# Keep-Passion/ImageStitch

Hardware: AMD Instinct MI355X
Metric: image-pairs/sec (2048x2048 grayscale, SURF+BF) (higher is better)
Workload: dtype f32

## Files before the change

### imagestitch_amd/csrc/match_kernels.hip

```cpp
#include "common.h"
#include <algorithm>
#include <stdlib.h>
#include <math.h>

typedef float float2v __attribute__((ext_vector_type(2)));
typedef const float __attribute__((address_space(4))) cfloat;
typedef float f16v __attribute__((ext_vector_type(16)));

#define SLOAD16(dst, ptr) asm volatile("s_load_dwordx16 %0, %1, 0x0" : "=s"(dst) : "s"(ptr))
#define SLOAD16_BEFORE(dst, ptr, live) asm volatile("s_load_dwordx16 %0, %2, 0x0" : "=s"(dst), "+s"(live) : "s"(ptr))
#define SWAIT(dst) asm volatile("s_waitcnt lgkmcnt(0)" : "+s"(dst))
#define SWAIT2(d0, d1) asm volatile("s_waitcnt lgkmcnt(0)" : "+s"(d0), "+s"(d1))
#define BF_CHUNK(buf, base)                                                                    \
    _Pragma("unroll") for (int d = 0; d < 16; d += 4) {                                        \
        float2v e0 = qv[base + d + 0] - buf[d + 0];                                            \
        float2v e1 = qv[base + d + 1] - buf[d + 1];                                            \
        float2v e2 = qv[base + d + 2] - buf[d + 2];                                            \
        float2v e3 = qv[base + d + 3] - buf[d + 3];                                            \
        acc += e0 * e0 + e1 * e1 + e2 * e2 + e3 * e3;                                          \
    }

__device__ __forceinline__ void knn_update(float dsq, int j, float &b1, float &b2, int &i1, float &b1sq, float &b2sq)
{
    if (dsq < b2sq) {
// ... 134 lines not shown
    float b1[4], b2[4], b1s[4], b2s[4];
#pragma unroll
    for (int u = 0; u < 4; u++) {
        const int q = qw + 16 * u + c;
        const i4v *qp = (const i4v *)(J.q8 + (size_t)q * 128);
        qb[u][0] = qp[g]; qb[u][1] = qp[4 + g];
        qn[u] = J.qn2[q];
        thr[u] = 0x7fffffff; i1[u] = -1;
        b1[u] = b2[u] = b1s[u] = b2s[u] = INFINITY;
    }
    for (int jt = t0; jt < t1; jt += 16) {
        const i4v *tp = (const i4v *)(J.t8 + (size_t)(jt + c) * 128);
        const i4v a0 = tp[g], a1 = tp[4 + g];
        const i4v tn = *(const i4v *)(J.tn2 + jt + 4 * g);
        const int j0 = jt + 4 * g;
#pragma unroll
        for (int u = 0; u < 4; u++) {
            i4v acc = {0, 0, 0, 0};
            acc = __builtin_amdgcn_mfma_i32_16x16x64_i8(a0, qb[u][0], acc, 0, 0, 0);
            acc = __builtin_amdgcn_mfma_i32_16x16x64_i8(a1, qb[u][1], acc, 0, 0, 0);
            const int s0 = tn[0] - 2 * acc[0], s1 = tn[1] - 2 * acc[1], s2 = tn[2] - 2 * acc[2], s3 = tn[3] - 2 * acc[3];
            if (min(min(s0, s1), min(s2, s3)) < thr[u]) {
                if (s0 < thr[u] && j0 < nt) knn_update((float)(s0 + qn[u]), j0, b1[u], b2[u], i1[u], b1s[u], b2s[u]);
                if (s1 < thr[u] && j0 + 1 < nt) knn_update((float)(s1 + qn[u]), j0 + 1, b1[u], b2[u], i1[u], b1s[u], b2s[u]);
                if (s2 < thr[u] && j0 + 2 < nt) knn_update((float)(s2 + qn[u]), j0 + 2, b1[u], b2[u], i1[u], b1s[u], b2s[u]);
                if (s3 < thr[u] && j0 + 3 < nt) knn_update((float)(s3 + qn[u]), j0 + 3, b1[u], b2[u], i1[u], b1s[u], b2s[u]);
                thr[u] = b2s[u] == INFINITY ? 0x7fffffff : (int)b2s[u] - qn[u];
            }
        }
    }
    const size_t o = (size_t)sp * J.capq;
#pragma unroll
    for (int u = 0; u < 4; u++) {
        float B1 = b1[u], B2 = b2[u]; int I1 = i1[u];
#pragma unroll
        for (int d = 16; d <= 32; d <<= 1) {
            const float ob1 = __shfl_xor(B1, d, 64), ob2 = __shfl_xor(B2, d, 64);
            const int oi1 = __shfl_xor(I1, d, 64);
            knn_merge(B1, B2, I1, ob1, ob2, oi1);
        }
        const int q = qw + 16 * u + c;
        if (g == 0 && q < nq) { J.p_d1[o + q] = B1; J.p_d2[o + q] = B2; J.p_i1[o + q] = I1; }
    }
}

#define BFM_CAPL 32
#define BFM_MARGIN 1e-3f
#define BFM_FAR 1e30f

struct BfmState { float m1, m2, thr; int cnt; };

__device__ __forceinline__ void bfm_warm(const f16v &acc, BfmState &S)
{
#pragma unroll
    for (int i = 0; i < 16; i++) {
        const float v = acc[i];
        S.m2 = fminf(S.m2, fmaxf(S.m1, v));
        S.m1 = fminf(S.m1, v);
    }
}
__device__ __forceinline__ void bfm_scan(const f16v &acc, BfmState &S, int row0, uint2 *list, size_t pitch, bool update)
{
#pragma unroll
    for (int i = 0; i < 16; i++) {
        const float v = acc[i];
        if (v <= S.thr && v < 1e29f) {
            if (S.cnt < BFM_CAPL) list[S.cnt * pitch] = make_uint2(__float_as_uint(v), (unsigned)(row0 + (i & 3) + 8 * (i >> 2)));
            S.cnt++;
            if (update) {
                S.m2 = fminf(S.m2, fmaxf(S.m1, v));
                S.m1 = fminf(S.m1, v);
                S.thr = S.m2 + BFM_MARGIN;
            }
        }
    }
}

__global__ __launch_bounds__(256, 2) void k_bf_mfma_d64(const MatchDev *jobs)
{
    const MatchDev &J = jobs[blockIdx.z];
    const int nq = __builtin_amdgcn_readfirstlane(*J.nq_ptr), nt = __builtin_amdgcn_readfirstlane(*J.nt_ptr);
    const int lane = threadIdx.x & 63, wave = threadIdx.x >> 6;
    const int q0 = (blockIdx.x * 4 + wave) * 64;
    if (q0 >= nq) return;
    const int nsplit = gridDim.y, sp = blockIdx.y;
    const int ntiles = (nt + 31) >> 5;
    const int tchunk = (ntiles + nsplit - 1) / nsplit;
    const int tile0 = sp * tchunk, tile1 = min(ntiles, tile0 + tchunk);
    const int col = lane & 31, half = lane >> 5;
    float bq0[32], bq1[32];
    {
        const float4 *p0 = reinterpret_cast<const float4 *>(J.q + (size_t)min(q0 + col, nq - 1) * 64 + 32 * half);
        const float4 *p1 = reinterpret_cast<const float4 *>(J.q + (size_t)min(q0 + 32 + col, nq - 1) * 64 + 32 * half);
#pragma unroll
        for (int s4 = 0; s4 < 8; s4++) {
            const float4 u = p0[s4], v = p1[s4];
            bq0[4 * s4 + 0] = -2.f * u.x; bq0[4 * s4 + 1] = -2.f * u.y; bq0[4 * s4 + 2] = -2.f * u.z; bq0[4 * s4 + 3] = -2.f * u.w;
            bq1[4 * s4 + 0] = -2.f * v.x; bq1[4 * s4 + 1] = -2.f * v.y; bq1[4 * s4 + 2] = -2.f * v.z; bq1[4 * s4 + 3] = -2.f * v.w;
        }
    }
    const float baug = half == 0 ? 1.f : 0.f;
    const bool va = q0 + col < nq, vb = q0 + 32 + col < nq;
    BfmState Sa = {INFINITY, INFINITY, INFINITY, 0}, Sb = {INFINITY, INFINITY, INFINITY, 0};
    const size_t pitch = (size_t)J.capq;
    const int lst = sp * 2 + half;
    uint2 *lista = J.c_ent + (size_t)lst * BFM_CAPL * pitch + (q0 + col), *listb = lista + 32;
    const float *T = J.t;
    for (int pass = 0; pass < 2; pass++) {
        const int tend = pass == 0 ? min(tile0 + 1, tile1) : tile1;
        float4 an[8];
        if (tile0 < tend) {
            const float4 *pn = reinterpret_cast<const float4 *>(T + (size_t)min(tile0 * 32 + col, nt - 1) * 64 + 32 * half);
#pragma unroll
            for (int s4 = 0; s4 < 8; s4++) an[s4] = pn[s4];
        }
        for (int tl = tile0; tl < tend; tl++) {
            float a[32];
#pragma unroll
            for (int s4 = 0; s4 < 8; s4++) { a[4 * s4] = an[s4].x; a[4 * s4 + 1] = an[s4].y; a[4 * s4 + 2] = an[s4].z; a[4 * s4 + 3] = an[s4].w; }
            if (tl + 1 < tend) {
                const float4 *pn = reinterpret_cast<const float4 *>(T + (size_t)min((tl + 1) * 32 + col, nt - 1) * 64 + 32 * half);
#pragma unroll
                for (int s4 = 0; s4 < 8; s4++) an[s4] = pn[s4];
            }
            float part = 0.f;
#pragma unroll
            for (int s = 0; s < 32; s++) part += a[s] * a[s];
            const float tnorm = part + __shfl_xor(part, 32, 64);
            const float aaug = half == 0 ? (tl * 32 + col < nt ? tnorm : BFM_FAR) : 0.f;
            f16v acc0 = {0, 0, 0, 0, 0, 0, 0, 0, 0, 0, 0, 0, 0, 0, 0, 0}, acc1 = acc0;
#pragma unroll
            for (int s = 0; s < 32; s++) {
                acc0 = __builtin_amdgcn_mfma_f32_32x32x2f32(a[s], bq0[s], acc0, 0, 0, 0);
                acc1 = __builtin_amdgcn_mfma_f32_32x32x2f32(a[s], bq1[s], acc1, 0, 0, 0);
            }
            acc0 = __builtin_amdgcn_mfma_f32_32x32x2f32(aaug, baug, acc0, 0, 0, 0);
            acc1 = __builtin_amdgcn_mfma_f32_32x32x2f32(aaug, baug, acc1, 0, 0, 0);
            if (pass == 0) {
                bfm_warm(acc0, Sa); bfm_warm(acc1, Sb);
            } else {
                const int row0 = tl * 32 + 4 * half;
                bfm_scan(acc0, Sa, row0, lista, pitch, tl != tile0); bfm_scan(acc1, Sb, row0, listb, pitch, tl != tile0);
            }
        }
        if (pass == 0) {
            Sa.thr = va ? Sa.m2 + BFM_MARGIN : -INFINITY;
            Sb.thr = vb ? Sb.m2 + BFM_MARGIN : -INFINITY;
        }
    }
    if (va) J.c_cnt[(size_t)lst * pitch + q0 + col] = Sa.cnt;
    if (vb) J.c_cnt[(size_t)lst * pitch + q0 + 32 + col] = Sb.cnt;
}

#define BF16_ROW 80
#define BF16_FRAGS 5
#define BFM_F16_ERR 2.0e-3f
typedef _Float16 h8v __attribute__((ext_vector_type(8)));

__global__ __launch_bounds__(256) void k_bf_split16(const MatchDev *jobs, float scale_q)
{
    const MatchDev &J = jobs[blockIdx.z];
    const bool is_t = blockIdx.y == 1;
    const int n = is_t ? *J.nt_ptr : *J.nq_ptr;
    const int row = blockIdx.x * 128 + (threadIdx.x >> 1), half = threadIdx.x & 1;
    if (row >= n) return;
    const float *src = (is_t ? J.t : J.q) + (size_t)row * 64 + 32 * half;
    const float sc = is_t ? 1.f : scale_q;
    float part = 0.f;
    h8v el[4];
#pragma unroll
    for (int d = 0; d < 32; d++) {
        const float x = src[d];
        part += x * x;
        el[d >> 3][d & 7] = (_Float16)(x * sc);
    }
    const float tot = part + __shfl_xor(part, 1, 64);
    h8v ns = {0, 0, 0, 0, 0, 0, 0, 0};
    if (half == 0) {
        _Float16 a = (_Float16)1.f, b = (_Float16)1.f;
        if (is_t) { a = (_Float16)tot; b = (_Float16)(tot - (float)a); }
        ns[0] = a; ns[1] = b;
    }
    if (is_t) {
        h8v *dst = reinterpret_cast<h8v *>(J.t16) + (size_t)(row >> 5) * (BF16_FRAGS * 64) + (row & 31) + 32 * half;
#pragma unroll
        for (int s4 = 0; s4 < 4; s4++) dst[s4 * 64] = el[s4];
        dst[4 * 64] = ns;
    } else {
        h8v *dst = reinterpret_cast<h8v *>(J.q16 + (size_t)row * BF16_ROW + 32 * half);
#pragma unroll
        for (int s4 = 0; s4 < 4; s4++) dst[s4] = el[s4];
        if (half == 0) *reinterpret_cast<h8v *>(J.q16 + (size_t)row * BF16_ROW + 64) = ns;
    }
}

#ifndef BFM_GLDS
#define BFM_GLDS 1
#endif
#define BFM_WINDOW (2.f * BFM_F16_ERR + BFM_MARGIN)
#define GASM __attribute__((address_space(1)))
typedef GASM const h8v *g_cs8v;
typedef float f2v __attribute__((ext_vector_type(2)));

#ifdef VFSMS_DESC_TIMING
__device__ unsigned long long g_bf_cycles[2][8];
extern "C" int vfsms_debug_bf_cycles(unsigned long long *out) { return hipMemcpyFromSymbol(out, HIP_SYMBOL(g_bf_cycles), sizeof(unsigned long long) * 16) == hipSuccess ? 0 : -3; }
#define BT_DECL unsigned long long _bt[5] = {0, 0, 0, 0, 0}, _bt0 = clock64(), _btl = _bt0
#define BT_MARK(ph) do { const unsigned long long _n = clock64(); _bt[ph] += _n - _btl; _btl = _n; } while (0)
#define BT_FLUSH(pass) do { if ((threadIdx.x & 63) == 0) { for (int _q = 0; _q < 5; _q++) atomicAdd(&g_bf_cycles[pass][_q], _bt[_q]); \
        atomicAdd(&g_bf_cycles[pass][5], clock64() - _bt0); atomicAdd(&g_bf_cycles[pass][6], 1ull); } } while (0)
#else
#define BT_DECL do {} while (0)
#define BT_MARK(ph) do {} while (0)
#define BT_FLUSH(pass) do {} while (0)
#endif
template <int PASS>
__global__ __launch_bounds__(256, 3) void k_bf_mfma16_d64(const MatchDev *jobs, int qblocks, int nsplit, int njobs)
{
    unsigned unit, qb;
    xcd_roi_map(blockIdx.x, (unsigned)qblocks, (unsigned)(nsplit * njobs), unit, qb);
    const int sp = (int)(unit % (unsigned)nsplit);
    const MatchDev &J = jobs[unit / (unsigned)nsplit];
    const int nq = __builtin_amdgcn_readfirstlane(*J.nq_ptr), nt = __builtin_amdgcn_readfirstlane(*J.nt_ptr);
    const int lane = threadIdx.x & 63, wave = threadIdx.x >> 6;
    if ((int)qb * 256 >= nq) return;
    BT_DECL;
    const int q0 = ((int)qb * 4 + wave) * 64;
    const bool live = q0 < nq;
    const int ntiles = (nt + 31) >> 5;
    const int tchunk = (ntiles + nsplit - 1) / nsplit;
    const int tile0 = sp * tchunk, tile1 = min(ntiles, tile0 + tchunk);
    const int col = lane & 31, half = lane >> 5;
    const h8v zero = {0, 0, 0, 0, 0, 0, 0, 0};
    h8v bh0[4], bh1[4], bn0, bn1;
    {
        g_cs8v p0 = (g_cs8v)(J.q16 + (size_t)min(q0 + col, nq - 1) * BF16_ROW + 32 * half);
        g_cs8v p1 = (g_cs8v)(J.q16 + (size_t)min(q0 + 32 + col, nq - 1) * BF16_ROW + 32 * half);
#pragma unroll
        for (int s4 = 0; s4 < 4; s4++) { bh0[s4] = p0[s4]; bh1[s4] = p1[s4]; }
        bn0 = half == 0 ? *(g_cs8v)(J.q16 + (size_t)min(q0 + col, nq - 1) * BF16_ROW + 64) : zero;
        bn1 = half == 0 ? *(g_cs8v)(J.q16 + (size_t)min(q0 + 32 + col, nq - 1) * BF16_ROW + 64) : zero;
    }
    constexpr int NFR = BF16_FRAGS;
    constexpr int BFM_UNIT = 2;
    __shared__ h8v stage[2][BFM_UNIT][NFR * 64];
    g_cs8v T = (g_cs8v)J.t16;
    const int tid = threadIdx.x; (void)tid;
#if BFM_GLDS
    constexpr int NSET = 1;
    const int wv_u = __builtin_amdgcn_readfirstlane(wave);
    auto glds16 = [&](g_cs8v src, const h8v *dst) {
        __builtin_amdgcn_global_load_lds((const __attribute__((address_space(1))) void *)src, (__attribute__((address_space(3))) void *)dst, 16, 0, 0);
    };
    auto fetch = [&](int unit, int b) {
#pragma unroll
        for (int u = 0; u < BFM_UNIT; u++) {
            const int tl = min(tile0 + unit * BFM_UNIT + u, tile1 - 1);
            g_cs8v pn = T + (size_t)tl * (BF16_FRAGS * 64);
            glds16(pn + 64 * wv_u + lane, &stage[b][u][64 * wv_u]);
            if (wv_u == 0) glds16(pn + 256 + lane, &stage[b][u][256]);
        }
    };
    const int nunits = (tile1 - tile0 + BFM_UNIT - 1) / BFM_UNIT;
    if (nunits > 0) fetch(0, 0);
#else
    constexpr int NSET = PASS == 0 ? 2 : 1;
    h8v g0[NSET][BFM_UNIT], g1[NSET][BFM_UNIT];
#pragma unroll
    for (int e = 0; e < NSET; e++)
#pragma unroll
        for (int u = 0; u < BFM_UNIT; u++) { g0[e][u] = zero; g1[e][u] = zero; }
    const int nunits = (tile1 - tile0 + BFM_UNIT - 1) / BFM_UNIT;
    auto fetch = [&](int unit, int e) {
#pragma unroll
        for (int u = 0; u < BFM_UNIT; u++) {
            const int tl = min(tile0 + unit * BFM_UNIT + u, tile1 - 1);
            g_cs8v pn = T + (size_t)tl * (BF16_FRAGS * 64);
            g0[e][u] = pn[tid];
            g1[e][u] = pn[256 + (tid & 63)];
        }
    };
    auto put = [&](int b, int e) {
#pragma unroll
        for (int u = 0; u < BFM_UNIT; u++) {
            stage[b][u][tid] = g0[e][u];
            if (tid < 64) stage[b][u][256 + tid] = g1[e][u];
        }
    };
    if (nunits > 0) fetch(0, 0);
#endif
#pragma unroll
    for (int s4 = 0; s4 < 4; s4++) asm volatile("" : "+v"(bh0[s4]), "+v"(bh1[s4]));
    asm volatile("" : "+v"(bn0), "+v"(bn1));
    const bool va = q0 + col < nq, vb = q0 + 32 + col < nq;
    const size_t pitch = (size_t)J.capq;
    const int lst = sp * 2 + half, nl = 2 * nsplit;
    float m1a = INFINITY, m2a = INFINITY, m1b = INFINITY, m2b = INFINITY;
    float thra = -INFINITY, thrb = -INFINITY;
    int cnta = 0, cntb = 0;
    if (PASS == 1) {
        GASM const f2v *B = (GASM const f2v *)J.c_m12;
        float a1 = INFINITY, a2 = INFINITY, b1 = INFINITY, b2 = INFINITY;
        for (int L0 = 0; L0 < nl; L0 += 4) {
            f2v ua[4], ub[4];
#pragma unroll
            for (int k = 0; k < 4; k++) {
                const size_t row = (size_t)min(L0 + k, nl - 1) * pitch;
                ua[k] = B[row + min(q0 + col, nq - 1)]; ub[k] = B[row + min(q0 + 32 + col, nq - 1)];
            }
#pragma unroll
            for (int k = 0; k < 4; k++) {
                if (L0 + k >= nl) break;
                a2 = fminf(fminf(a2, ua[k].y), fmaxf(a1, ua[k].x)); a1 = fminf(a1, ua[k].x);
                b2 = fminf(fminf(b2, ub[k].y), fmaxf(b1, ub[k].x)); b1 = fminf(b1, ub[k].x);
            }
        }
        if (va) thra = a2 + BFM_WINDOW;
        if (vb) thrb = b2 + BFM_WINDOW;
    }
    GASM unsigned long long *lista = (GASM unsigned long long *)J.c_ent + (size_t)lst * BFM_CAPL * pitch + (q0 + col), *listb = lista + 32;
#if !BFM_GLDS
    if (nunits > 0) {
        put(0, 0);
#pragma unroll
        for (int k = 1; k <= NSET; k++) fetch(min(k, nunits - 1), k % NSET);
    }
#endif
    BT_MARK(0);
    for (int unit0 = 0; unit0 < nunits; unit0 += NSET) {
#pragma unroll
      for (int v = 0; v < NSET; v++) {
        const int unit = unit0 + v;
        if (unit >= nunits) break;
        const int b = unit & 1;
#if BFM_GLDS
        asm volatile("s_waitcnt vmcnt(0)" ::: "memory");
#endif
        __syncthreads();
        BT_MARK(1);
#if BFM_GLDS
        if (unit + 1 < nunits) fetch(unit + 1, b ^ 1);
#else
        if (unit + 1 < nunits) put(b ^ 1, (v + 1) % NSET);
        fetch(min(unit + 1 + NSET, nunits - 1), (v + 1) % NSET);
#endif
        BT_MARK(2);
        if (!live) continue;
#pragma unroll
        for (int u = 0; u < BFM_UNIT; u++) {
            const int tl = tile0 + unit * BFM_UNIT + u;
            if (tl >= tile1) break;
            const h8v *st = stage[b][u];
            f16v acc0 = {0, 0, 0, 0, 0, 0, 0, 0, 0, 0, 0, 0, 0, 0, 0, 0}, acc1 = acc0;
#pragma unroll
            for (int s = 0; s < 4; s++) {
                const h8v at = st[s * 64 + lane];
                acc0 = __builtin_amdgcn_mfma_f32_32x32x16_f16(at, bh0[s], acc0, 0, 0, 0);
                acc1 = __builtin_amdgcn_mfma_f32_32x32x16_f16(at, bh1[s], acc1, 0, 0, 0);
            }
            const h8v na = st[(NFR - 1) * 64 + lane];
            acc0 = __builtin_amdgcn_mfma_f32_32x32x16_f16(na, bn0, acc0, 0, 0, 0);
            acc1 = __builtin_amdgcn_mfma_f32_32x32x16_f16(na, bn1, acc1, 0, 0, 0);
            if (tl * 32 + 31 >= nt) {
#pragma unroll
                for (int i = 0; i < 16; i++) {
                    const bool past = tl * 32 + 4 * half + (i & 3) + 8 * (i >> 2) >= nt;
                    acc0[i] = past ? BFM_FAR : acc0[i]; acc1[i] = past ? BFM_FAR : acc1[i];
                }
            }
            if (PASS == 0) {
                float ta = fminf(fminf(acc0[0], acc0[1]), fminf(acc0[2], acc0[3])), tb = fminf(fminf(acc1[0], acc1[1]), fminf(acc1[2], acc1[3]));
#pragma unroll
                for (int i = 4; i < 16; i += 3) {
                    ta = fminf(ta, fminf(acc0[i], fminf(acc0[i + 1], acc0[i + 2])));
                    tb = fminf(tb, fminf(acc1[i], fminf(acc1[i + 1], acc1[i + 2])));
                }
                m2a = fminf(m2a, fmaxf(m1a, ta)); m1a = fminf(m1a, ta);
                m2b = fminf(m2b, fmaxf(m1b, tb)); m1b = fminf(m1b, tb);
            } else {
                const int row0 = tl * 32 + 4 * half;
#pragma unroll
                for (int h = 0; h < 2; h++) {
                    const f16v &acc = h == 0 ? acc0 : acc1;
                    const float thr = h == 0 ? thra : thrb;
                    float gm[5];
                    gm[0] = fminf(fminf(acc[0], acc[1]), fminf(acc[2], acc[3]));
#pragma unroll
                    for (int g = 1; g < 5; g++) gm[g] = fminf(acc[3 * g + 1], fminf(acc[3 * g + 2], acc[3 * g + 3]));
                    const float mn = fminf(fminf(gm[0], fminf(gm[1], gm[2])), fminf(gm[3], gm[4]));
                    const bool some = __any(mn <= thr);
                    BT_MARK(3);
                    if (some) {
                        GASM unsigned long long *list = h == 0 ? lista : listb;
                        int cnt = h == 0 ? cnta : cntb;
#pragma unroll
                        for (int g = 0; g < 5; g++) {
                            if (!__any(gm[g] <= thr)) continue;
#pragma unroll
                            for (int i = (g == 0 ? 0 : 3 * g + 1); i < (g == 0 ? 4 : 3 * g + 4); i++) {
                                const float v = acc[i];
                                if (v <= thr && v < 1e29f) {
                                    if (cnt < BFM_CAPL) list[cnt * pitch] = (unsigned long long)__float_as_uint(v) | ((unsigned long long)(unsigned)(row0 + (i & 3) + 8 * (i >> 2)) << 32);
                                    cnt++;
                                }
                            }
                        }
                        if (h == 0) cnta = cnt; else cntb = cnt;
                        BT_MARK(4);
                    }
                }
            }
            if (PASS == 0) BT_MARK(3);
        }
      }
    }
    BT_FLUSH(PASS);
    if (PASS == 0) {
        GASM f2v *B = (GASM f2v *)J.c_m12;
        if (va) B[(size_t)lst * pitch + q0 + col] = f2v{m1a, m2a};
        if (vb) B[(size_t)lst * pitch + q0 + 32 + col] = f2v{m1b, m2b};
    } else {
        if (va) J.c_cnt[(size_t)lst * pitch + q0 + col] = cnta;
        if (vb) J.c_cnt[(size_t)lst * pitch + q0 + 32 + col] = cntb;
    }
}

#define BFV_HITS 12
#ifdef VFSMS_DESC_TIMING
__device__ unsigned g_bfv_stats[4];
extern "C" int vfsms_debug_bfv_stats(unsigned *out) { return hipMemcpyFromSymbol(out, HIP_SYMBOL(g_bfv_stats), sizeof(unsigned) * 4) == hipSuccess ? 0 : -3; }
#define BFV_STAT(i, v) atomicAdd(&g_bfv_stats[i], (unsigned)(v))
#else
#define BFV_STAT(i, v) do {} while (0)
#endif
__device__ __forceinline__ void bfv_exact(const float *__restrict__ Qr, const float *__restrict__ T, int idx, float &B1, float &B2, int &I1)
{
    const float4 *tr = reinterpret_cast<const float4 *>(T + (size_t)idx * 64);
    const float4 *qr = reinterpret_cast<const float4 *>(Qr);
    float acc = 0.f;
#pragma unroll
    for (int d4 = 0; d4 < 16; d4++) {
        const float4 tv = tr[d4], qv = qr[d4];
        const float e0 = qv.x - tv.x, e1 = qv.y - tv.y, e2 = qv.z - tv.z, e3 = qv.w - tv.w;
        acc += e0 * e0 + e1 * e1 + e2 * e2 + e3 * e3;
    }
    const float d = sqrtf(acc);
    if (d < B1 || (d == B1 && idx < I1)) { B2 = B1; B1 = d; I1 = idx; }
    else B2 = fminf(B2, d);
}

__global__ __launch_bounds__(256) void k_bf_verify_d64(const MatchDev *jobs, int cns, float window)
{
    const MatchDev &J = jobs[blockIdx.y];
    const int nq = __builtin_amdgcn_readfirstlane(*J.nq_ptr), nt = __builtin_amdgcn_readfirstlane(*J.nt_ptr);
    if ((int)(blockIdx.x * 256) >= nq) return;
    const int q = blockIdx.x * 256 + threadIdx.x;
    const bool live = q < nq;
    const int nl = 2 * cns;
    const size_t pitch = (size_t)J.capq;
    __shared__ int hits[BFV_HITS][256];
    float s1 = INFINITY, s2 = INFINITY; bool overflow = false;
    if (live)
        for (int L = 0; L < nl; L++) {
            const int c = J.c_cnt[(size_t)L * pitch + q];
            overflow = overflow || c > BFM_CAPL;
            BFV_STAT(2, min(c, BFM_CAPL));
            const uint2 *e = J.c_ent + (size_t)L * BFM_CAPL * pitch + q;
            for (int k = 0; k < min(c, BFM_CAPL); k++) {
                const float v = __uint_as_float(e[k * pitch].x);
                s2 = fminf(s2, fmaxf(s1, v));
                s1 = fminf(s1, v);
            }
        }
    const float cut = s2 + window;
    if (live) { BFV_STAT(0, 1); BFV_STAT(1, overflow ? 1 : 0); }
    const float *Qr = J.q + (size_t)min(q, nq - 1) * 64;
    float B1 = INFINITY, B2 = INFINITY; int I1 = -1;
    int nh = 0;
    if (live && !overflow)
        for (int L = 0; L < nl; L++) {
            const int c = min(J.c_cnt[(size_t)L * pitch + q], BFM_CAPL);
            const uint2 *e = J.c_ent + (size_t)L * BFM_CAPL * pitch + q;
            for (int k = 0; k < c; k++) {
                const uint2 ev = e[k * pitch];
                if (__uint_as_float(ev.x) <= cut) {
                    if (nh < BFV_HITS) hits[nh++][threadIdx.x] = (int)ev.y;
                    else bfv_exact(Qr, J.t, (int)ev.y, B1, B2, I1);
                }
            }
        }
    if (live) BFV_STAT(3, nh);
    int maxh = nh;
#pragma unroll
    for (int d = 32; d >= 1; d >>= 1) maxh = max(maxh, __shfl_xor(maxh, d, 64));
    for (int k = 0; k < maxh; k++)
        if (k < nh) bfv_exact(Qr, J.t, hits[k][threadIdx.x], B1, B2, I1);
    {
        const int lane = threadIdx.x & 63;
        unsigned long long om = __ballot(live && overflow);
        while (om) {
            const int src = __ffsll((long long)om) - 1;
            om &= om - 1;
            const int qo = __shfl(q, src, 64);
            const float *Qo = J.q + (size_t)qo * 64;
            float b1 = INFINITY, b2 = INFINITY; int i1 = -1;
            for (int j = lane; j < nt; j += 64) bfv_exact(Qo, J.t, j, b1, b2, i1);
#pragma unroll
            for (int d = 32; d >= 1; d >>= 1) {
                const float ob1 = __shfl_xor(b1, d, 64), ob2 = __shfl_xor(b2, d, 64);
                const int oi1 = __shfl_xor(i1, d, 64);
                if (ob1 < b1 || (ob1 == b1 && oi1 >= 0 && (i1 < 0 || oi1 < i1))) { b2 = fminf(b1, ob2); b1 = ob1; i1 = oi1; }
                else b2 = fminf(b2, ob1);
            }
            if (lane == src) { B1 = b1; B2 = b2; I1 = i1; }
        }
    }
    if (live) { J.p_d1[q] = B1; J.p_d2[q] = B2; J.p_i1[q] = I1; }
}

__global__ __launch_bounds__(256) void k_merge_ratio(const MatchDev *jobs, double ratio, int do_ratio)
{
    const MatchDev &J = jobs[blockIdx.y];
    const int nq = __builtin_amdgcn_readfirstlane(*J.nq_ptr), nt = __builtin_amdgcn_readfirstlane(*J.nt_ptr);
    const int q = blockIdx.x * 256 + threadIdx.x;
    if (q >= nq) return;
    float B1 = INFINITY, B2 = INFINITY; int I1 = -1;
    for (int s = 0; s < J.nsplit; s++) {
        const size_t o = (size_t)s * J.capq + q;
        float d = J.p_d1[o]; int i = J.p_i1[o];
        if (i >= 0) {
            if (d < B1) { B2 = B1; B1 = d; I1 = i; } else if (d < B2) { B2 = d; }
            float e = J.p_d2[o];
            if (e < B1) { B2 = B1; B1 = e; } else if (e < B2) { B2 = e; }
        }
    }
    J.d1[q] = B1; J.d2[q] = B2; J.i1[q] = I1;
    if (!do_ratio) return;
    int ok = (I1 >= 0) && (nt >= 2) && ((double)B1 < (double)B2 * ratio);
    int vote = 0;
    if (ok && J.kq) {
        float ay = J.kq[2 * q + 1], ax = J.kq[2 * q];
        float by = J.kt[2 * I1 + 1], bx = J.kt[2 * I1];
        int dx = (int)(ay - by), dy = (int)(ax - bx);
        vote = !(dx == 0 && dy == 0);
        J.votes[2 * (size_t)(J.capq + q)] = dx;
        J.votes[2 * (size_t)(J.capq + q) + 1] = dy;
    }
    J.match_flag[q] = ok | (vote << 1);
}

__device__ __forceinline__ int wave_incl_scan_i(int v)
{
    const int lane = threadIdx.x & 63;
#pragma unroll
    for (int d = 1; d < 64; d <<= 1) {
        int n = __shfl_up(v, d, 64);
        if (lane >= d) v += n;
    }
    return v;
}

__global__ __launch_bounds__(1024) void k_match_scan(const MatchDev *jobs)
{
    const MatchDev &J = jobs[blockIdx.x];
    const int nq = *J.nq_ptr;
    __shared__ int wsum_m[16], wsum_v[16];
    __shared__ int carry_m, carry_v;
// ... 50 lines not shown
    __shared__ int wsum_m[16], wsum_v[16];
    __shared__ int carry_m, carry_v;
    __shared__ uint32_t hkey[MODE_SLOTS], hcnt[MODE_SLOTS], hfirst[MODE_SLOTS];
    __shared__ unsigned long long best;
    if (threadIdx.x == 0) { carry_m = 0; carry_v = 0; best = 0ull; }
    for (int s = threadIdx.x; s < MODE_SLOTS; s += 1024) { hkey[s] = 0u; hcnt[s] = 0u; hfirst[s] = 0xFFFFFFFFu; }
    __syncthreads();
    const int lane = threadIdx.x & 63, wid = threadIdx.x >> 6;
    for (int base = 0; base < nq; base += 1024) {
        const int q = base + threadIdx.x;
        const int f = (q < nq) ? J.match_flag[q] : 0;
        const int fm = f & 1, fv = (f >> 1) & 1;
        const int im = wave_incl_scan_i(fm), iv = wave_incl_scan_i(fv);
        if (lane == 63) { wsum_m[wid] = im; wsum_v[wid] = iv; }
        __syncthreads();
        int om = carry_m, ov = carry_v;
        for (int k = 0; k < wid; k++) { om += wsum_m[k]; ov += wsum_v[k]; }
        if (fm && !J.pairs_given) {
            const int pos = om + im - 1;
            J.pairs[2 * (size_t)pos] = J.i1[q];
            J.pairs[2 * (size_t)pos + 1] = q;
        }
        if (fv) {
            const int pos = ov + iv - 1;
            J.votes[2 * (size_t)pos] = J.votes[2 * (size_t)(J.capq + q)];
            J.votes[2 * (size_t)pos + 1] = J.votes[2 * (size_t)(J.capq + q) + 1];
        }
        __syncthreads();
        if (threadIdx.x == 1023) { carry_m = om + im; carry_v = ov + iv; }
        __syncthreads();
    }
    const int nm = carry_m, nv = carry_v;
    if (threadIdx.x == 0) { J.mcount[0] = nm; J.mcount[1] = nv; J.mcount[2] = 0; J.mcount[3] = 0; }
    __threadfence_block();
    __syncthreads();
    const int P = (nv + MODE_HASH_MAX - 1) / MODE_HASH_MAX;
    for (int pass = 0; pass < P; pass++) {
        if (pass > 0) {
            __syncthreads();
            for (int s = threadIdx.x; s < MODE_SLOTS; s += 1024) { hkey[s] = 0u; hcnt[s] = 0u; hfirst[s] = 0xFFFFFFFFu; }
            __syncthreads();
        }
        for (int i = threadIdx.x; i < nv; i += 1024) {
            const int dx = J.votes[2 * (size_t)i], dy = J.votes[2 * (size_t)i + 1];
            const uint32_t key = ((uint32_t)(dx + 32768) << 16) | ((uint32_t)(dy + 32768) & 0xffffu);
            if (P > 1 && (int)(((key ^ (key >> 15)) * 0x9E3779B1u >> 8) % (uint32_t)P) != pass) continue;
            uint32_t h = (key * 2654435761u) >> 19;
            for (;;) {
                const uint32_t old = atomicCAS(&hkey[h], 0u, key);
                if (old == 0u || old == key) { atomicAdd(&hcnt[h], 1u); atomicMin(&hfirst[h], (uint32_t)i); break; }
                h = (h + 1) & (MODE_SLOTS - 1);
            }
        }
        __syncthreads();
        unsigned long long mine = 0ull;
        for (int s = threadIdx.x; s < MODE_SLOTS; s += 1024)
            if (hcnt[s]) {
                const unsigned long long bid = ((unsigned long long)hcnt[s] << 32) | (unsigned long long)(0xFFFFFFFFu - hfirst[s]);
                mine = bid > mine ? bid : mine;
            }
        for (int d = 32; d > 0; d >>= 1) { const unsigned long long o = __shfl_down(mine, d, 64); mine = o > mine ? o : mine; }
        if (lane == 0 && mine) atomicMax(&best, mine);
    }
    __syncthreads();
    if (threadIdx.x == 0) {
        int status = 0, dx = 0, dy = 0, votes = 0;
        if (nm > 0) {
            if (nv == 0) { votes = 1; }
            else {
                votes = (int)(best >> 32);
                const unsigned idx = 0xFFFFFFFFu - (unsigned)(best & 0xFFFFFFFFull);
                dx = J.votes[2 * (size_t)idx]; dy = J.votes[2 * (size_t)idx + 1];
            }
            status = votes >= offset_evaluate;
        }
        *reinterpret_cast<unsigned long long *>(J.mcount + 2) = best;
        J.result[0] = status; J.result[1] = dx; J.result[2] = dy; J.result[3] = votes;
        J.result[4] = *J.nq_ptr; J.result[5] = *J.nt_ptr; J.result[6] = nm; J.result[7] = 0;
    }
}

__global__ __launch_bounds__(256) void k_bf_hamming32(const uint32_t *__restrict__ q, int nq,
                                                      const uint32_t *__restrict__ t, int nt,
                                                      int *best_idx, int *best_dist)
{
    const int qi = blockIdx.x * 256 + threadIdx.x;
    if (blockIdx.x * 256 >= nq) return;
    const uint32_t *pq = q + (size_t)min(qi, nq - 1) * 8;
    uint32_t v[8];
#pragma unroll
    for (int k = 0; k < 8; k++) v[k] = pq[k];
    int best = 0x7fffffff, bi = -1;
    for (int j = 0; j < nt; j++) {
        const uint32_t *__restrict__ tr = t + (size_t)j * 8;
        int d = 0;
#pragma unroll
        for (int k = 0; k < 8; k++) d += __popc(v[k] ^ tr[k]);
        if (d < best) { best = d; bi = j; }
    }
    if (qi < nq) { best_idx[qi] = bi; best_dist[qi] = best; }
}

static inline size_t al(size_t x) { return (x + 255) & ~(size_t)255; }

size_t match_bytes(int capq, int nsplit)
{
    size_t b = 3 * al(sizeof(float) * (size_t)capq * nsplit);
    b += 3 * al(sizeof(float) * capq) + 2 * al(sizeof(int) * capq);
    b += al(sizeof(int32_t) * 2 * capq) + al(sizeof(int32_t) * 4 * capq) + al(64) + al(64) + al(64);
    return b + 4096;
}

int match_carve(vfsms_ctx *ctx, MatchDev *m, int capq, int dim, int nsplit)
{
    m->capq = capq; m->dim = dim; m->nsplit = nsplit;
    m->p_d1 = (float *)ctx_arena_alloc(ctx, sizeof(float) * (size_t)capq * nsplit);
    m->p_d2 = (float *)ctx_arena_alloc(ctx, sizeof(float) * (size_t)capq * nsplit);
    m->p_i1 = (int *)ctx_arena_alloc(ctx, sizeof(int) * (size_t)capq * nsplit);
    m->d1 = (float *)ctx_arena_alloc(ctx, sizeof(float) * capq);
    m->d2 = (float *)ctx_arena_alloc(ctx, sizeof(float) * capq);
    m->i1 = (int *)ctx_arena_alloc(ctx, sizeof(int) * capq);
    m->match_flag = (int *)ctx_arena_alloc(ctx, sizeof(int) * capq);
    m->match_pos = (int *)ctx_arena_alloc(ctx, sizeof(int) * capq);
    m->pairs = (int32_t *)ctx_arena_alloc(ctx, sizeof(int32_t) * 2 * capq);
    m->votes = (int32_t *)ctx_arena_alloc(ctx, sizeof(int32_t) * 4 * capq);
    m->mcount = (int *)ctx_arena_alloc(ctx, 64);
    m->vsum = (unsigned long long *)ctx_arena_alloc(ctx, 64);
    m->result = (int32_t *)ctx_arena_alloc(ctx, 64);
    if (!m->result) { vfsms_set_error("arena exhausted while carving a match job"); return VFSMS_ERR_CAPACITY; }
    return VFSMS_OK;
}

__global__ __launch_bounds__(256) void k_max_norm2_d64(const float *a, int n, unsigned *out)
{
    const int row = blockIdx.x * 4 + (threadIdx.x >> 6), lane = threadIdx.x & 63;
    if (row >= n) return;
    const float v = a[(size_t)row * 64 + lane];
    float s = v * v;
#pragma unroll
    for (int d = 32; d >= 1; d >>= 1) s += __shfl_xor(s, d, 64);
    if (lane == 0) atomicMax(out, __float_as_uint(s == s ? s : INFINITY));
}

int launch_max_norm2_d64(vfsms_ctx *ctx, const float *a, int n, unsigned *d_out)
{
    if (n > 0) hipLaunchKernelGGL(k_max_norm2_d64, dim3((n + 3) / 4), dim3(256), 0, ctx->stream, a, n, d_out);
    HIP_TRY(hipGetLastError());
    return VFSMS_OK;
}

size_t match_filter_bytes(int capq, int capt, int cns)
{
    return al(sizeof(uint2) * (size_t)capq * cns * 2 * BFM_CAPL) + al(sizeof(int) * (size_t)capq * cns * 2) +
           al(sizeof(unsigned short) * BF16_ROW * (size_t)capq) + al(sizeof(unsigned short) * BF16_ROW * ((size_t)capt + 32)) +
           al(sizeof(float2) * (size_t)capq * cns * 2) + 1024;
}

int match_filter_carve(vfsms_ctx *ctx, MatchDev *m, int capq, int capt, int cns)
{
    m->c_ent = (uint2 *)ctx_arena_alloc(ctx, sizeof(uint2) * (size_t)capq * cns * 2 * BFM_CAPL);
    m->c_cnt = (int *)ctx_arena_alloc(ctx, sizeof(int) * (size_t)capq * cns * 2);
    m->q16 = (unsigned short *)ctx_arena_alloc(ctx, sizeof(unsigned short) * BF16_ROW * (size_t)capq);
    m->t16 = (unsigned short *)ctx_arena_alloc(ctx, sizeof(unsigned short) * BF16_ROW * ((size_t)capt + 32));
    m->c_m12 = (float2 *)ctx_arena_alloc(ctx, sizeof(float2) * (size_t)capq * cns * 2);
    if (!m->c_cnt || !m->t16 || !m->c_m12) { vfsms_set_error("arena exhausted while carving a match filter"); return VFSMS_ERR_CAPACITY; }
    return VFSMS_OK;
}

static bool bf_f32_filter()
{
    static const bool v = getenv("VFSMS_BF_F32FILTER") && atoi(getenv("VFSMS_BF_F32FILTER")) != 0;
    return v;
}

int launch_bf_l2_filtered(vfsms_ctx *ctx, const MatchDev *d_jobs, int njobs, int capq, int capt, int cns)
{
    if (njobs <= 0 || capq <= 0) return VFSMS_OK;
    {
        ProfScope ps(ctx, "bf_mfma");
        if (bf_f32_filter())
            hipLaunchKernelGGL(k_bf_mfma_d64, dim3((capq + 255) / 256, cns, njobs), dim3(256), 0, ctx->stream, d_jobs);
        else {
            hipLaunchKernelGGL(k_bf_split16, dim3((std::max(capq, capt) + 127) / 128, 2, njobs), dim3(256), 0, ctx->stream, d_jobs, -2.f);
            const int qblocks = (capq + 255) / 256;
            hipLaunchKernelGGL(k_bf_mfma16_d64<0>, dim3((unsigned)qblocks * cns * njobs), dim3(256), 0, ctx->stream, d_jobs, qblocks, cns, njobs);
            hipLaunchKernelGGL(k_bf_mfma16_d64<1>, dim3((unsigned)qblocks * cns * njobs), dim3(256), 0, ctx->stream, d_jobs, qblocks, cns, njobs);
        }
    }
    {
        ProfScope ps(ctx, "bf_verify");
        hipLaunchKernelGGL(k_bf_verify_d64, dim3((capq + 255) / 256, njobs), dim3(256), 0, ctx->stream, d_jobs, cns, bf_f32_filter() ? BFM_MARGIN : BFM_WINDOW);
    }
    HIP_TRY(hipGetLastError());
    return VFSMS_OK;
}

int launch_bf_l2(vfsms_ctx *ctx, const MatchDev *d_jobs, int njobs, int capq, int nsplit, int dim)
{
    if (njobs <= 0 || capq <= 0) return VFSMS_OK;
    ProfScope ps(ctx, "bf_l2");
    if (dim == 64) {
        hipLaunchKernelGGL(k_bf_l2_d64, dim3((capq + 511) / 512, nsplit, njobs), dim3(256), 0, ctx->stream, d_jobs);
    } else if (dim == 128) {
        hipLaunchKernelGGL(k_bf_l2_gen<128>, dim3((capq + 255) / 256, nsplit, njobs), dim3(256), 0, ctx->stream, d_jobs);
    } else if (dim == 32) {
        hipLaunchKernelGGL(k_bf_l2_gen<32>, dim3((capq + 255) / 256, nsplit, njobs), dim3(256), 0, ctx->stream, d_jobs);
    } else {
        vfsms_set_error("bf_l2: descriptor dim %d unsupported (64, 128, 32)", dim);
        return VFSMS_ERR_UNSUPPORTED;
    }
    HIP_TRY(hipGetLastError());
    return VFSMS_OK;
}

int launch_pack_i8_d128(vfsms_ctx *ctx, const PackJob *d_jobs, int njobs, int max_rows)
{
    if (njobs <= 0 || max_rows <= 0) return VFSMS_OK;
    ProfScope ps(ctx, "pack_i8");
    hipLaunchKernelGGL(k_pack_i8_d128, dim3((max_rows + 63) / 64, njobs), dim3(256), 0, ctx->stream, d_jobs);
    HIP_TRY(hipGetLastError());
    return VFSMS_OK;
}

int launch_bf_i8_d128(vfsms_ctx *ctx, const MatchDev *d_jobs, int njobs, int capq, int nsplit)
{
    if (njobs <= 0 || capq <= 0) return VFSMS_OK;
    ProfScope ps(ctx, "bf_i8");
    hipLaunchKernelGGL(k_bf_i8_d128, dim3((capq + 255) / 256, nsplit, njobs), dim3(256), 0, ctx->stream, d_jobs);
    HIP_TRY(hipGetLastError());
    return VFSMS_OK;
}

static int launch_vote_tail(vfsms_ctx *ctx, const MatchDev *d_jobs, int njobs, int capq, int estimator, int tol, int offset_evaluate)
{
    if (estimator == VFSMS_OFFSET_CONSENSUS) {
        hipLaunchKernelGGL(k_match_scan, dim3(njobs), dim3(1024), 0, ctx->stream, d_jobs);
        HIP_TRY(hipGetLastError());
        return launch_consensus(ctx, d_jobs, njobs, capq, tol, offset_evaluate);
    }
    hipLaunchKernelGGL(k_scan_mode, dim3(njobs), dim3(1024), 0, ctx->stream, d_jobs, offset_evaluate);
    HIP_TRY(hipGetLastError());
    return VFSMS_OK;
}

static int verify_tail(vfsms_ctx *ctx, const MatchDev *d_jobs, int njobs)
{
    if (ctx->offset_verifier != VFSMS_VERIFY_NCC) return VFSMS_OK;
    return launch_verify(ctx, d_jobs, njobs, ctx->verify_threshold, ctx->verify_min_pixels);
}

int launch_ratio_mode(vfsms_ctx *ctx, const MatchDev *d_jobs, int njobs, int capq, double ratio, int offset_evaluate)
{
    if (njobs <= 0) return VFSMS_OK;
    {
        ProfScope ps(ctx, "vote");
        hipLaunchKernelGGL(k_merge_ratio, dim3((capq + 255) / 256, njobs), dim3(256), 0, ctx->stream, d_jobs, ratio, 1);
        TRY(launch_vote_tail(ctx, d_jobs, njobs, capq, ctx->offset_estimator, ctx->offset_tol, offset_evaluate));
    }
    return verify_tail(ctx, d_jobs, njobs);
}

int launch_ratio_only(vfsms_ctx *ctx, const MatchDev *d_jobs, int njobs, int capq, double ratio)
{
    hipLaunchKernelGGL(k_merge_ratio, dim3((capq + 255) / 256, njobs), dim3(256), 0, ctx->stream, d_jobs, ratio, 1);
    hipLaunchKernelGGL(k_match_scan, dim3(njobs), dim3(1024), 0, ctx->stream, d_jobs);
    HIP_TRY(hipGetLastError());
    return VFSMS_OK;
}

int launch_merge_only(vfsms_ctx *ctx, const MatchDev *d_jobs, int njobs, int capq)
{
    hipLaunchKernelGGL(k_merge_ratio, dim3((capq + 255) / 256, njobs), dim3(256), 0, ctx->stream, d_jobs, 0.0, 0);
    HIP_TRY(hipGetLastError());
    return VFSMS_OK;
}

int launch_scan_mode(vfsms_ctx *ctx, const MatchDev *d_jobs, int njobs, int capq, int offset_evaluate)
{
    if (njobs <= 0) return VFSMS_OK;
    {
        ProfScope ps(ctx, "vote");
        TRY(launch_vote_tail(ctx, d_jobs, njobs, capq, ctx->offset_estimator, ctx->offset_tol, offset_evaluate));
    }
    return verify_tail(ctx, d_jobs, njobs);
}

int launch_mode_only(vfsms_ctx *ctx, const MatchDev *d_jobs, int njobs, int capm, int estimator, int tol, int offset_evaluate)
{
    if (njobs <= 0) return VFSMS_OK;
    if (capm > 0)
        hipLaunchKernelGGL(k_votes_from_pairs, dim3((capm + 255) / 256, njobs), dim3(256), 0, ctx->stream, d_jobs, capm);
    return launch_vote_tail(ctx, d_jobs, njobs, capm, estimator, tol, offset_evaluate);
}

int launch_bf_hamming(vfsms_ctx *ctx, const uint8_t *q, int nq, const uint8_t *t, int nt, int nbytes,
                      int *best_idx, int *best_dist)
{
    if (nbytes != 32) { vfsms_set_error("bf_hamming: only 32-byte descriptors supported"); return VFSMS_ERR_UNSUPPORTED; }
    if (nq <= 0) return VFSMS_OK;
    hipLaunchKernelGGL(k_bf_hamming32, dim3((nq + 255) / 256), dim3(256), 0, ctx->stream,
                       (const uint32_t *)q, nq, (const uint32_t *)t, nt, best_idx, best_dist);
    HIP_TRY(hipGetLastError());
    return VFSMS_OK;
}
```

Measured before the change: 2451.

## Fold train norms into MFMA accumulator init and subsample tiles in threshold pass

Result: faster. 2480, median of 6 (+1.2%).

```diff
diff --git a/imagestitch_amd/csrc/match_kernels.hip b/imagestitch_amd/csrc/match_kernels.hip
--- a/imagestitch_amd/csrc/match_kernels.hip
+++ b/imagestitch_amd/csrc/match_kernels.hip
@@ -310,8 +310,9 @@
     if (vb) J.c_cnt[(size_t)lst * pitch + q0 + 32 + col] = Sb.cnt;
 }
 
-#define BF16_ROW 80
-#define BF16_FRAGS 5
+#define BF16_ROW 64
+#define BF16_FRAGS 4
+#define BF16_TILE (BF16_FRAGS * 64 + 8)
 #define BFM_F16_ERR 2.0e-3f
 typedef _Float16 h8v __attribute__((ext_vector_type(8)));
 
@@ -332,28 +333,22 @@
         part += x * x;
         el[d >> 3][d & 7] = (_Float16)(x * sc);
     }
-    const float tot = part + __shfl_xor(part, 1, 64);
-    h8v ns = {0, 0, 0, 0, 0, 0, 0, 0};
-    if (half == 0) {
-        _Float16 a = (_Float16)1.f, b = (_Float16)1.f;
-        if (is_t) { a = (_Float16)tot; b = (_Float16)(tot - (float)a); }
-        ns[0] = a; ns[1] = b;
-    }
     if (is_t) {
-        h8v *dst = reinterpret_cast<h8v *>(J.t16) + (size_t)(row >> 5) * (BF16_FRAGS * 64) + (row & 31) + 32 * half;
+        h8v *tile = reinterpret_cast<h8v *>(J.t16) + (size_t)(row >> 5) * BF16_TILE;
+        h8v *dst = tile + (row & 31) + 32 * half;
 #pragma unroll
         for (int s4 = 0; s4 < 4; s4++) dst[s4 * 64] = el[s4];
-        dst[4 * 64] = ns;
+        const float tot = part + __shfl_xor(part, 1, 64);
+        if (half == 0) reinterpret_cast<float *>(tile + BF16_FRAGS * 64)[row & 31] = tot;
     } else {
         h8v *dst = reinterpret_cast<h8v *>(J.q16 + (size_t)row * BF16_ROW + 32 * half);
 #pragma unroll
         for (int s4 = 0; s4 < 4; s4++) dst[s4] = el[s4];
-        if (half == 0) *reinterpret_cast<h8v *>(J.q16 + (size_t)row * BF16_ROW + 64) = ns;
-    }
-}
-
-#ifndef BFM_GLDS
-#define BFM_GLDS 1
+    }
+}
+
+#ifndef BFM_P0_STRIDE
+#define BFM_P0_STRIDE 2
 #endif
 #define BFM_WINDOW (2.f * BFM_F16_ERR + BFM_MARGIN)
 #define GASM __attribute__((address_space(1)))
@@ -375,6 +370,7 @@
 template <int PASS>
 __global__ __launch_bounds__(256, 3) void k_bf_mfma16_d64(const MatchDev *jobs, int qblocks, int nsplit, int njobs)
 {
+    static_assert(BFM_P0_STRIDE == 1 || BFM_P0_STRIDE == 2 || BFM_P0_STRIDE == 4, "BFM_P0_STRIDE is 1, 2 or 4");
     unsigned unit, qb;
     xcd_roi_map(blockIdx.x, (unsigned)qblocks, (unsigned)(nsplit * njobs), unit, qb);
     const int sp = (int)(unit % (unsigned)nsplit);
@@ -388,68 +384,36 @@
     const int ntiles = (nt + 31) >> 5;
     const int tchunk = (ntiles + nsplit - 1) / nsplit;
     const int tile0 = sp * tchunk, tile1 = min(ntiles, tile0 + tchunk);
+    constexpr int STRIDE = PASS == 0 ? BFM_P0_STRIDE : 1;
+    const int nvis = tile1 > tile0 ? (tile1 - tile0 - 1 + STRIDE - 1) / STRIDE + 1 : 0;
+    auto tile_of = [&](int k) { return min(tile0 + k * STRIDE, tile1 - 1); };
     const int col = lane & 31, half = lane >> 5;
-    const h8v zero = {0, 0, 0, 0, 0, 0, 0, 0};
-    h8v bh0[4], bh1[4], bn0, bn1;
+    h8v bh0[4], bh1[4];
     {
         g_cs8v p0 = (g_cs8v)(J.q16 + (size_t)min(q0 + col, nq - 1) * BF16_ROW + 32 * half);
         g_cs8v p1 = (g_cs8v)(J.q16 + (size_t)min(q0 + 32 + col, nq - 1) * BF16_ROW + 32 * half);
 #pragma unroll
         for (int s4 = 0; s4 < 4; s4++) { bh0[s4] = p0[s4]; bh1[s4] = p1[s4]; }
-        bn0 = half == 0 ? *(g_cs8v)(J.q16 + (size_t)min(q0 + col, nq - 1) * BF16_ROW + 64) : zero;
-        bn1 = half == 0 ? *(g_cs8v)(J.q16 + (size_t)min(q0 + 32 + col, nq - 1) * BF16_ROW + 64) : zero;
-    }
-    constexpr int NFR = BF16_FRAGS;
+    }
     constexpr int BFM_UNIT = 2;
-    __shared__ h8v stage[2][BFM_UNIT][NFR * 64];
+    __shared__ h8v stage[2][BFM_UNIT][BF16_TILE];
     g_cs8v T = (g_cs8v)J.t16;
-    const int tid = threadIdx.x; (void)tid;
-#if BFM_GLDS
-    constexpr int NSET = 1;
     const int wv_u = __builtin_amdgcn_readfirstlane(wave);
     auto glds16 = [&](g_cs8v src, const h8v *dst) {
         __builtin_amdgcn_global_load_lds((const __attribute__((address_space(1))) void *)src, (__attribute__((address_space(3))) void *)dst, 16, 0, 0);
     };
+    const int nunits = (nvis + BFM_UNIT - 1) / BFM_UNIT;
     auto fetch = [&](int unit, int b) {
 #pragma unroll
         for (int u = 0; u < BFM_UNIT; u++) {
-            const int tl = min(tile0 + unit * BFM_UNIT + u, tile1 - 1);
-            g_cs8v pn = T + (size_t)tl * (BF16_FRAGS * 64);
+            g_cs8v pn = T + (size_t)tile_of(min(unit * BFM_UNIT + u, nvis - 1)) * BF16_TILE;
             glds16(pn + 64 * wv_u + lane, &stage[b][u][64 * wv_u]);
-            if (wv_u == 0) glds16(pn + 256 + lane, &stage[b][u][256]);
-        }
-    };
-    const int nunits = (tile1 - tile0 + BFM_UNIT - 1) / BFM_UNIT;
-    if (nunits > 0) fetch(0, 0);
-#else
-    constexpr int NSET = PASS == 0 ? 2 : 1;
-    h8v g0[NSET][BFM_UNIT], g1[NSET][BFM_UNIT];
-#pragma unroll
-    for (int e = 0; e < NSET; e++)
-#pragma unroll
-        for (int u = 0; u < BFM_UNIT; u++) { g0[e][u] = zero; g1[e][u] = zero; }
-    const int nunits = (tile1 - tile0 + BFM_UNIT - 1) / BFM_UNIT;
-    auto fetch = [&](int unit, int e) {
-#pragma unroll
-        for (int u = 0; u < BFM_UNIT; u++) {
-            const int tl = min(tile0 + unit * BFM_UNIT + u, tile1 - 1);
-            g_cs8v pn = T + (size_t)tl * (BF16_FRAGS * 64);
-            g0[e][u] = pn[tid];
-            g1[e][u] = pn[256 + (tid & 63)];
-        }
-    };
-    auto put = [&](int b, int e) {
-#pragma unroll
-        for (int u = 0; u < BFM_UNIT; u++) {
-            stage[b][u][tid] = g0[e][u];
-            if (tid < 64) stage[b][u][256 + tid] = g1[e][u];
+            if (wv_u == 0 && lane < 8) glds16(pn + BF16_FRAGS * 64 + lane, &stage[b][u][BF16_FRAGS * 64]);
         }
     };
     if (nunits > 0) fetch(0, 0);
-#endif
 #pragma unroll
     for (int s4 = 0; s4 < 4; s4++) asm volatile("" : "+v"(bh0[s4]), "+v"(bh1[s4]));
-    asm volatile("" : "+v"(bn0), "+v"(bn1));
     const bool va = q0 + col < nq, vb = q0 + 32 + col < nq;
     const size_t pitch = (size_t)J.capq;
     const int lst = sp * 2 + half, nl = 2 * nsplit;
@@ -477,48 +441,36 @@
         if (vb) thrb = b2 + BFM_WINDOW;
     }
     GASM unsigned long long *lista = (GASM unsigned long long *)J.c_ent + (size_t)lst * BFM_CAPL * pitch + (q0 + col), *listb = lista + 32;
-#if !BFM_GLDS
-    if (nunits > 0) {
-        put(0, 0);
-#pragma unroll
-        for (int k = 1; k <= NSET; k++) fetch(min(k, nunits - 1), k % NSET);
-    }
-#endif
     BT_MARK(0);
-    for (int unit0 = 0; unit0 < nunits; unit0 += NSET) {
-#pragma unroll
-      for (int v = 0; v < NSET; v++) {
-        const int unit = unit0 + v;
-        if (unit >= nunits) break;
+    for (int unit = 0; unit < nunits; unit++) {
         const int b = unit & 1;
-#if BFM_GLDS
         asm volatile("s_waitcnt vmcnt(0)" ::: "memory");
-#endif
         __syncthreads();
         BT_MARK(1);
-#if BFM_GLDS
         if (unit + 1 < nunits) fetch(unit + 1, b ^ 1);
-#else
-        if (unit + 1 < nunits) put(b ^ 1, (v + 1) % NSET);
-        fetch(min(unit + 1 + NSET, nunits - 1), (v + 1) % NSET);
-#endif
         BT_MARK(2);
         if (!live) continue;
 #pragma unroll
         for (int u = 0; u < BFM_UNIT; u++) {
-            const int tl = tile0 + unit * BFM_UNIT + u;
-            if (tl >= tile1) break;
+            if (unit * BFM_UNIT + u >= nvis) break;
+            const int tl = tile_of(unit * BFM_UNIT + u);
             const h8v *st = stage[b][u];
-            f16v acc0 = {0, 0, 0, 0, 0, 0, 0, 0, 0, 0, 0, 0, 0, 0, 0, 0}, acc1 = acc0;
-#pragma unroll
-            for (int s = 0; s < 4; s++) {
+            const float4 *tn = reinterpret_cast<const float4 *>(st + BF16_FRAGS * 64) + half;
+            f16v cinit;
+#pragma unroll
+            for (int j = 0; j < 4; j++) {
+                const float4 n4 = tn[2 * j];
+                cinit[4 * j] = n4.x; cinit[4 * j + 1] = n4.y; cinit[4 * j + 2] = n4.z; cinit[4 * j + 3] = n4.w;
+            }
+            const h8v at0 = st[lane];
+            f16v acc0 = __builtin_amdgcn_mfma_f32_32x32x16_f16(at0, bh0[0], cinit, 0, 0, 0);
+            f16v acc1 = __builtin_amdgcn_mfma_f32_32x32x16_f16(at0, bh1[0], cinit, 0, 0, 0);
+#pragma unroll
+            for (int s = 1; s < 4; s++) {
                 const h8v at = st[s * 64 + lane];
                 acc0 = __builtin_amdgcn_mfma_f32_32x32x16_f16(at, bh0[s], acc0, 0, 0, 0);
                 acc1 = __builtin_amdgcn_mfma_f32_32x32x16_f16(at, bh1[s], acc1, 0, 0, 0);
             }
-            const h8v na = st[(NFR - 1) * 64 + lane];
-            acc0 = __builtin_amdgcn_mfma_f32_32x32x16_f16(na, bn0, acc0, 0, 0, 0);
-            acc1 = __builtin_amdgcn_mfma_f32_32x32x16_f16(na, bn1, acc1, 0, 0, 0);
             if (tl * 32 + 31 >= nt) {
 #pragma unroll
                 for (int i = 0; i < 16; i++) {
@@ -570,7 +522,6 @@
             }
             if (PASS == 0) BT_MARK(3);
         }
-      }
     }
     BT_FLUSH(PASS);
     if (PASS == 0) {
@@ -927,7 +878,7 @@
 size_t match_filter_bytes(int capq, int capt, int cns)
 {
     return al(sizeof(uint2) * (size_t)capq * cns * 2 * BFM_CAPL) + al(sizeof(int) * (size_t)capq * cns * 2) +
-           al(sizeof(unsigned short) * BF16_ROW * (size_t)capq) + al(sizeof(unsigned short) * BF16_ROW * ((size_t)capt + 32)) +
+           al(sizeof(unsigned short) * BF16_ROW * (size_t)capq) + al(sizeof(h8v) * BF16_TILE * ((size_t)capt / 32 + 1)) +
            al(sizeof(float2) * (size_t)capq * cns * 2) + 1024;
 }
 
@@ -936,7 +887,7 @@
     m->c_ent = (uint2 *)ctx_arena_alloc(ctx, sizeof(uint2) * (size_t)capq * cns * 2 * BFM_CAPL);
     m->c_cnt = (int *)ctx_arena_alloc(ctx, sizeof(int) * (size_t)capq * cns * 2);
     m->q16 = (unsigned short *)ctx_arena_alloc(ctx, sizeof(unsigned short) * BF16_ROW * (size_t)capq);
-    m->t16 = (unsigned short *)ctx_arena_alloc(ctx, sizeof(unsigned short) * BF16_ROW * ((size_t)capt + 32));
+    m->t16 = (unsigned short *)ctx_arena_alloc(ctx, sizeof(h8v) * BF16_TILE * ((size_t)capt / 32 + 1));
     m->c_m12 = (float2 *)ctx_arena_alloc(ctx, sizeof(float2) * (size_t)capq * cns * 2);
     if (!m->c_cnt || !m->t16 || !m->c_m12) { vfsms_set_error("arena exhausted while carving a match filter"); return VFSMS_ERR_CAPACITY; }
     return VFSMS_OK;
```
